# romi2002/gym-usv

Hardware: AMD Instinct MI355X
Metric: env-steps/sec at 65 536 parallel envs; 1/2/4/8 MI355X scaling (higher is better)
Workload: dtype f32; 1 GPU; C3: usv-simple, 65536 envs per GPU, random-action rollout, in-kernel TimeLimit + same-step autoreset; env_id=usv-simple, envs_per_gpu=65536, global_envs=65536, parallelism=env-sharded x1, no step-path collective, lidar=window

## Files before the change

gym-usv_amd/csrc/usv_kernels.hip:

```cpp
#include <hip/hip_runtime.h>

#include <algorithm>
#include <cstdio>
#include <type_traits>
#include <cstdlib>
#include <cstring>
#include <string>
#include <vector>

#include "usv_device.hpp"
#include "usv_hip.h"

namespace usv {

template <typename R> struct V4;
template <> struct V4<float> { typedef float T __attribute__((ext_vector_type(4))); };
template <> struct V4<double> { typedef double T __attribute__((ext_vector_type(4))); };
template <typename R> using R4 = typename V4<R>::T;

enum RealField {
  F_X, F_Y, F_PSI, F_U, F_V, F_R, F_LAST_U, F_LAST_R, F_PROGRESS,
  F_PX0, F_PY0, F_PX1, F_PY1, F_MAX_U, F_MAX_R, F_REF_V, F_NREAL
};

// ... 48 lines not shown
  }
}
constexpr int kExpN = 0, kExpPS = 1, kExpAngle = 3, kExpPose = 4, kExpObs = 8;

template <typename R> struct IO {
  const float* act;
  float* obs;
  R* rew;
  uint8_t* term;
  uint8_t* trunc;
  float* fobs;
  const uint8_t* mask;
  R* info;
  int kpath;
  uint8_t* done;
};

constexpr int kBlock = 256;
constexpr int kWaves = kBlock / kWave;
constexpr int kEPBReset = 64;
constexpr int kLidDefault = 7;

template <typename R> __device__ __forceinline__ R big() { return R(1e30); }

#ifdef USV_DIAG
#include "usv_diag.hpp"
#else
#define USV_STAMP_ID() do {} while (0)
#define USV_STAMP(i) do {} while (0)
#define USV_STAMP_B(i) do {} while (0)
#define USV_STAMP_W(i) do {} while (0)
#define USV_STAMP_V(i, v) do {} while (0)
struct Prof {
  __device__ void mark(int) {}
  __device__ void count(int) {}
  __device__ void flush(int) {}
};
struct QProf { __device__ void mark(int) {} __device__ void count(int, unsigned = 1) {} __device__ void flush() {} };
#define QMARK(i) do {} while (0)
#define QCOUNT(i, k) do {} while (0)
__device__ __forceinline__ void qprof_flush(QProf*) {}
#endif
template <typename T> __device__ __forceinline__ void st_out(T* p, T v) {
  __hip_atomic_store(p, v, __ATOMIC_RELAXED, __HIP_MEMORY_SCOPE_AGENT);
}
template <typename T> __device__ __forceinline__ void st_obs(T* p, T v) { st_out(p, v); }

constexpr int kRowSpanFrom = 196608;
constexpr int kStaticPrio = 1;

template <typename R> __device__ __forceinline__ R dyn_div(R a, R b) { return a / b; }
template <typename R> __device__ __forceinline__ R dyn_sqrt(R x) { return m_sqrt(x); }
template <> __device__ __forceinline__ float dyn_div(float a, float b) { return a * __builtin_amdgcn_rcpf(b); }
template <> __device__ __forceinline__ float dyn_sqrt(float x) { return __builtin_amdgcn_sqrtf(x); }

template <typename R> struct Vec2;
template <> struct Vec2<float> { using T = float2; };
template <> struct Vec2<double> { using T = double2; };

template <typename R> __device__ __forceinline__ R cdiv(R x, double c) { return div_const(x, c); }
template <> __device__ __forceinline__ float cdiv(float x, double c) { return x * (float)(1.0 / c); }

template <typename R>
__device__ __forceinline__ void make_header(float (&h)[kHdr], R u, R v, R r, R angle, R dist,
                                            R ye, R refv, R act_u, R act_r, R mu, R mr) {
  h[0] = (float)cdiv(u, 10); h[1] = (float)cdiv(v, 10); h[2] = (float)cdiv(r, 10);
  h[3] = (float)cdiv(angle, kPi); h[4] = (float)cdiv(dist, kDiag);
  h[5] = (float)cdiv(ye, 10); h[6] = (float)cdiv(refv, 10);
  h[7] = (float)dyn_div(act_u, mu); h[8] = (float)dyn_div(act_r, mr);
  h[9] = (float)cdiv(mu, 10); h[10] = 0.0f; h[11] = (float)cdiv(mr, 10);
  h[12] = (float)(kMaxAccU / 10.0); h[13] = 0.0f; h[14] = (float)(kMaxAccR / 10.0);
}

template <typename R> struct Uni4 { R u[4]; };
__device__ __forceinline__ void philox_uniforms(Philox& g, int l, Uni4<float>& o) {
  uint32_t a[4];
  g.c3 = (uint32_t)l;
  g.block(a[0], a[1], a[2], a[3]);
#pragma unroll
  for (int i = 0; i < 4; ++i) o.u[i] = (float)(a[i] >> 8) * (1.0f / 16777216.0f);
}
__device__ __forceinline__ void philox_uniforms(Philox& g, int l, Uni4<double>& o) {
  uint32_t a[4], b[4];
  g.c3 = (uint32_t)l;
  g.block(a[0], a[1], a[2], a[3]);
  g.c3 = (uint32_t)l + 64u;
  g.block(b[0], b[1], b[2], b[3]);
  const double k = 1.0 / 9007199254740992.0;
  o.u[0] = (double)((((uint64_t)a[0] << 32) | a[1]) >> 11) * k;
  o.u[1] = (double)((((uint64_t)a[2] << 32) | a[3]) >> 11) * k;
  o.u[2] = (double)((((uint64_t)b[0] << 32) | b[1]) >> 11) * k;
  o.u[3] = (double)((((uint64_t)b[2] << 32) | b[3]) >> 11) * k;
}

template <typename R>
__device__ __forceinline__ void reset_info(R* info, R x, R y, R psi, R u, R v, R r, R px0, R py0,
                                           R px1, R py1, R ye, R angle_n) {
  const R vals[USV_INFO_DIM] = {x, y, psi, u, v, r, px0, py0, px1, py1, R(0), R(0),
                                ye, angle_n, R(0), R(0), R(0), R(0), R(0), R(0), R(0), R(0)};
#pragma unroll
  for (int i = 0; i < USV_INFO_DIM; ++i) info[i] = vals[i];
}

template <typename R>
__device__ __forceinline__ R path_ye(R x, R y, R x0, R y0, R x1, R y1) {
  const R dx = x1 - x0, dy = y1 - y0;
  const R inv_len = R(1) / m_sqrt(dx * dx + dy * dy);
  return -(x - x0) * (dy * inv_len) + (y - y0) * (dx * inv_len);
}

template <typename R>
__device__ __forceinline__ void reset_experiment(const State<R>& S, int e, int ep, float* row, R* info) {
  const R* X = S.exp;
  R tx, ty, u, v, r, mu, mr, refv;
  {
    Philox g(S.seed, S.gid0 + (uint64_t)e, (uint32_t)ep);
    Uni4<R> U33, U34, U35;
    philox_uniforms(g, 33, U33);
    philox_uniforms(g, 34, U34);
    philox_uniforms(g, 35, U35);
    tx = R(kBound) * U33.u[1]; ty = R(kBound) * U33.u[2];
    u = R(0.15) * U33.u[3]; v = R(0.15) * U34.u[0]; r = R(0.15) * U34.u[1];
    mu = R(1.5) + R(1.5) * U34.u[2];
    mr = R(3) + R(3) * U34.u[3];
    refv = R(0.75) + (mu - R(0.75)) * U35.u[0];
  }
  const int cnt = (int)X[kExpN];
  R* ob = S.orow(e);
  for (int j = 0; j < S.cap; ++j) {
    ob[j] = j < cnt ? X[kExpObs + j] : R(0);
    ob[S.ostride + j] = j < cnt ? X[kExpObs + S.cap + j] : R(0);
    ob[2 * S.ostride + j] = j < cnt ? X[kExpObs + 2 * S.cap + j] : R(0);
  }
  const R ps0 = X[kExpPS], ps1 = X[kExpPS + 1];
  R sx2, cx2;
  m_sincos(X[kExpAngle], &sx2, &cx2);
  const R pe0 = ps0 + cx2 * R(100), pe1 = ps1 + sx2 * R(100);
  const R px = X[kExpPose], py = X[kExpPose + 1], psi = X[kExpPose + 2];
  S.F(F_X)[e] = px; S.F(F_Y)[e] = py;
  store_heading<R>(S, e, psi);
  S.F(F_PX0)[e] = ps0; S.F(F_PY0)[e] = ps1;
  S.F(F_PX1)[e] = pe0; S.F(F_PY1)[e] = pe1;
  S.I(I_NOBS)[e] = cnt;
  const R angle = wrap_angle(m_atan2(ty - py, tx - px) - psi);
  const R dst = m_hypot(px - tx, py - ty);
  const R ye = path_ye(px, py, ps0, ps1, pe0, pe1);
  float h[kHdr];
  make_header<R>(h, u, v, r, angle, dst, ye, refv, R(0), R(0), mu, mr);
  for (int i = 0; i < kHdr; ++i) row[i] = h[i];
  if (info) reset_info<R>(info, px, py, psi, u, v, r, ps0, ps1, pe0, pe1, ye, cdiv(angle, kPi));
}

template <typename R, int MODE>
__device__ __forceinline__ void reset_wave(const State<R>& S, int e, float* row, R* info = nullptr,
                                           int kpath = 0) {
  if (S.np_reset) return;
  const int l = lane_id();
  const int ep = uniform(S.I(I_EPISODE)[e]);
  Philox g(S.seed, S.gid0 + (uint64_t)e, (uint32_t)ep);
  Uni4<R> U;
  philox_uniforms(g, l, U);
  const R bm = m_sqrt(R(-2) * log(R(1) - bcast(U.u[0], 32)));
  R sb, cb;
  m_sincos(R(2 * kPi) * bcast(U.u[1], 32), &sb, &cb);
  const R sx = R(kBound / 2) + R(0.5) * bm * cb, sy = R(kBound / 2) + R(0.5) * bm * sb;
  const R tx = R(kBound) * bcast(U.u[1], 33), ty = R(kBound) * bcast(U.u[2], 33);
  const R mu = R(1.5) + R(1.5) * bcast(U.u[2], 34);
  const int n = min(15 + (int)(bcast(U.u[1], 35) * R(15)), 29);
  const R ox = R(kBound) * U.u[0], oy = R(kBound) * U.u[1], orad = R(0.15) + R(0.35) * U.u[2];
  const bool keep = (l < n) && !(m_hypot(sx - ox, sy - oy) < R(0.5) || m_hypot(tx - ox, ty - oy) < R(0.5));
  const unsigned long long ball = ballot(keep);
  int cnt = __popcll(ball);
  const int pos = __builtin_amdgcn_mbcnt_hi((unsigned)(ball >> 32), __builtin_amdgcn_mbcnt_lo((unsigned)ball, 0));
  R* ob = S.orow(e);
  const int os = S.ostride;
  if (keep) { ob[pos] = ox; ob[os + pos] = oy; ob[2 * os + pos] = orad; }
  if (cnt == 0) {
    const R fx = R(kBound) * bcast(U.u[2], 35), fy = R(kBound) * bcast(U.u[3], 35);
    const R fr = R(0.15) + R(0.35) * bcast(U.u[0], 36);
    if (l == 0) { ob[0] = fx; ob[os] = fy; ob[2 * os] = fr; }
    cnt = 1;
  }
  const R ang = R(-kPi) + R(2 * kPi) * bcast(U.u[3], 32);
  if (kpath > 0) {
    R sa, ca;
    m_sincos(ang, &sa, &ca);
    Uni4<R> P;
    philox_uniforms(g, l + 128, P);
    const R mag = R(kBound) * P.u[0];
    const R bq = m_sqrt(R(-2) * log(R(1) - P.u[1]));
    R s2, c2;
    m_sincos(R(2 * kPi) * P.u[2], &s2, &c2);
    const R lx = (ca * mag + sx) + bq * c2, ly = (sa * mag + sy) + bq * s2;
    const R lr = R(0.15) + R(0.35) * P.u[3];
    if (l < kpath) { ob[cnt + l] = lx; ob[os + cnt + l] = ly; ob[2 * os + cnt + l] = lr; }
    cnt += kpath;
  }
  if (l >= cnt && l < S.cap) { ob[l] = R(0); ob[os + l] = R(0); ob[2 * os + l] = R(0); }
  if (MODE == USV_MODE_ASMC_SIMPLE && l < kAsmcN) S.asmc[(size_t)l * S.N + e] = R(0);
  if (l == 0) {
    const R psi = R(-kPi) + R(2 * kPi) * bcast(U.u[2], 32);
    const R dist = R(100) + R(10) * bcast(U.u[0], 33);
    const R u = R(0.15) * bcast(U.u[3], 33), v = R(0.15) * bcast(U.u[0], 34), r = R(0.15) * bcast(U.u[1], 34);
    const R mr = R(3) + R(3) * bcast(U.u[3], 34);
    const R refv = R(0.75) + (mu - R(0.75)) * bcast(U.u[0], 35);
    R sa, ca;
    m_sincos(ang, &sa, &ca);
    S.F(F_X)[e] = sx; S.F(F_Y)[e] = sy;
    store_heading<R>(S, e, psi);
    S.F(F_U)[e] = u; S.F(F_V)[e] = v; S.F(F_R)[e] = r;
    S.F(F_PROGRESS)[e] = R(0);
    S.F(F_PX0)[e] = sx; S.F(F_PY0)[e] = sy;
    S.F(F_PX1)[e] = sx + ca * dist; S.F(F_PY1)[e] = sy + sa * dist;
    S.F(F_MAX_U)[e] = mu; S.F(F_MAX_R)[e] = mr; S.F(F_REF_V)[e] = refv;
    S.I(I_NOBS)[e] = cnt;
    S.I(I_ELAPSED)[e] = 0;
    S.I(I_EPISODE)[e] = ep + 1;
    S.I(I_SCAN)[e] = 0;
    const R angle = wrap_angle(m_atan2(ty - sy, tx - sx) - psi);
    const R dst = m_hypot(sx - tx, sy - ty);
    float h[kHdr];
    make_header<R>(h, u, v, r, angle, dst, R(0), refv, R(0), R(0), mu, mr);
#pragma unroll
    for (int i = 0; i < kHdr; ++i) row[i] = h[i];
    if (info) reset_info<R>(info, sx, sy, psi, u, v, r, sx, sy, sx + ca * dist, sy + sa * dist, R(0), cdiv(angle, kPi));
  }
}

template <typename R> __device__ __forceinline__ void heading_sincos(R psi, R* s, R* c) { fx_sincos(psi, s, c); }


#include "np_ziggurat.inc"
struct NpPcg64 {
  uint64_t sh, sl, ih, il;
  uint32_t has32, u32;
  __device__ uint64_t next64() {
    constexpr uint64_t kMh = 2549297995355413924ULL, kMl = 4865540595714422341ULL;
    const uint64_t lo = sl * kMl;
    const uint64_t hi = __umul64hi(sl, kMl) + sl * kMh + sh * kMl;
    const uint64_t nlo = lo + il;
    sh = hi + ih + (nlo < lo ? 1ULL : 0ULL);
    sl = nlo;
    const uint64_t x = sh ^ sl;
    const unsigned rot = (unsigned)(sh >> 58);
    return (x >> rot) | (x << ((64u - rot) & 63u));
  }
  __device__ uint32_t next32() {
    if (has32) { has32 = 0; return u32; }
    const uint64_t v = next64();
    has32 = 1;
    u32 = (uint32_t)(v >> 32);
    return (uint32_t)v;
  }
  __device__ double next_double() { return (double)(next64() >> 11) * (1.0 / 9007199254740992.0); }
  __device__ double standard_normal() {
    constexpr double kR = 3.6541528853610088, kInvR = 0.27366123732975828;
    for (;;) {
      uint64_t r = next64();
      const int idx = (int)(r & 0xff);
      r >>= 8;
      const bool neg = r & 1;
      const uint64_t rabs = (r >> 1) & 0x000fffffffffffffULL;
      double x = (double)rabs * kNpZigWi[idx];
      if (neg) x = -x;
      if (rabs < kNpZigKi[idx]) return x;
      if (idx == 0) {
        for (;;) {
          const double xx = -kInvR * log1p(-next_double());
          const double yy = -log1p(-next_double());
          if (yy + yy > xx * xx) return ((rabs >> 8) & 1) ? -(kR + xx) : kR + xx;
        }
      }
      if ((kNpZigFi[idx - 1] - kNpZigFi[idx]) * next_double() + kNpZigFi[idx] < exp(-0.5 * x * x)) return x;
    }
  }
  __device__ double uniform(double lo, double hi) { return lo + (hi - lo) * next_double(); }
  __device__ int integers(int lo, int hi) {
    const uint32_t rng = (uint32_t)(hi - 1 - lo), excl = rng + 1;
    uint64_t m = (uint64_t)next32() * excl;
    uint32_t left = (uint32_t)m;
    if (left < excl) {
      const uint32_t thr = (0xFFFFFFFFu - rng) % excl;
      while (left < thr) { m = (uint64_t)next32() * excl; left = (uint32_t)m; }
    }
    return lo + (int)(m >> 32);
  }
};

template <typename R>
__device__ __forceinline__ NpPcg64 np_load(const State<R>& S, int e) {
  auto w = [&](int i) { return (uint64_t)S.nprng[(size_t)i * S.fstride + e]; };
  return NpPcg64{w(0) | (w(1) << 32), w(2) | (w(3) << 32), w(4) | (w(5) << 32), w(6) | (w(7) << 32),
                 (uint32_t)w(8), (uint32_t)w(9)};
}
template <typename R>
__device__ __forceinline__ void np_store(const State<R>& S, int e, const NpPcg64& g) {
  const uint32_t v[10] = {(uint32_t)g.sh, (uint32_t)(g.sh >> 32), (uint32_t)g.sl, (uint32_t)(g.sl >> 32),
                          (uint32_t)g.ih, (uint32_t)(g.ih >> 32), (uint32_t)g.il, (uint32_t)(g.il >> 32),
                          g.has32, g.u32};
  for (int i = 0; i < 10; ++i) S.nprng[(size_t)i * S.fstride + e] = v[i];
}

template <typename R, int MODE>
__device__ void np_reset(const State<R>& S, int e, float* row, R* info = nullptr, int kpath = 0) {
  NpPcg64 g = np_load(S, e);
  const double sx = 0.5 * g.standard_normal() + kBound / 2;
  const double sy = 0.5 * g.standard_normal() + kBound / 2;
  (void)g.standard_normal(); (void)g.standard_normal(); (void)g.next_double();
  const double psi = g.uniform(-kPi, kPi);
  const double ang = g.uniform(-kPi, kPi), dist = g.uniform(100, 110);
  const double tx = g.uniform(0, kBound), ty = g.uniform(0, kBound);
  const double u = g.uniform(0.0, 0.15), v = g.uniform(0.0, 0.15), r = g.uniform(0.0, 0.15);
  const double mu = g.uniform(1.50, 3);
  (void)g.next_double(); (void)g.next_double();
  const double mr = g.uniform(3, 6);
  const double refv = g.uniform(0.75, mu);
  const int n = g.integers(15, 30);
  R* ob = S.orow(e);
  const int os = S.ostride;
  int cnt = 0;
  for (int j = 0; j < n; ++j) {
    const double ox = g.uniform(0, kBound), oy = g.uniform(0, kBound);
    if (!(hypot(sx - ox, sy - oy) < 0.5 || hypot(tx - ox, ty - oy) < 0.5)) {
      ob[cnt] = R(ox); ob[os + cnt] = R(oy); ++cnt;
    }
  }
  if (cnt == 0) {
    const double ox = g.uniform(0, kBound), oy = g.uniform(0, kBound);
    ob[0] = R(ox); ob[os] = R(oy); cnt = 1;
  }
  if (kpath > 0) {
    const double ca = cos(ang), sa = sin(ang);
    NpPcg64 gx = g, gy = g;
    for (int j = 0; j < kpath; ++j) (void)g.next_double();
    for (int j = 0; j < kpath; ++j) ob[cnt + j] = R((ca * gx.uniform(0, kBound) + sx) + g.standard_normal());
    for (int j = 0; j < kpath; ++j) ob[os + cnt + j] = R((sa * gy.uniform(0, kBound) + sy) + g.standard_normal());
    cnt += kpath;
  }
  for (int j = 0; j < cnt; ++j) ob[2 * os + j] = R(g.uniform(0.15, 0.5));
  np_store(S, e, g);
  double ps0 = sx, ps1 = sy, pe0 = sx + cos(ang) * dist, pe1 = sy + sin(ang) * dist;
  double px = sx, py = sy, pp = psi;
  if (const R* X = S.exp) {
    cnt = (int)X[kExpN];
    for (int j = 0; j < cnt; ++j) {
      ob[j] = X[kExpObs + j]; ob[os + j] = X[kExpObs + S.cap + j]; ob[2 * os + j] = X[kExpObs + 2 * S.cap + j];
    }
    ps0 = (double)X[kExpPS]; ps1 = (double)X[kExpPS + 1];
    pe0 = ps0 + cos((double)X[kExpAngle]) * 100; pe1 = ps1 + sin((double)X[kExpAngle]) * 100;
    px = (double)X[kExpPose]; py = (double)X[kExpPose + 1]; pp = (double)X[kExpPose + 2];
  }
  for (int j = cnt; j < S.cap; ++j) { ob[j] = R(0); ob[os + j] = R(0); ob[2 * os + j] = R(0); }
  if (MODE == USV_MODE_ASMC_SIMPLE)
    for (int i = 0; i < kAsmcN; ++i) S.asmc[(size_t)i * S.N + e] = R(0);
  const R x0 = R(px), y0 = R(py), ps = R(pp);
  S.F(F_X)[e] = x0; S.F(F_Y)[e] = y0;
  store_heading<R>(S, e, ps);
  S.F(F_U)[e] = R(u); S.F(F_V)[e] = R(v); S.F(F_R)[e] = R(r);
  S.F(F_PROGRESS)[e] = R(0);
  S.F(F_PX0)[e] = R(ps0); S.F(F_PY0)[e] = R(ps1);
  S.F(F_PX1)[e] = R(pe0); S.F(F_PY1)[e] = R(pe1);
  S.F(F_MAX_U)[e] = R(mu); S.F(F_MAX_R)[e] = R(mr); S.F(F_REF_V)[e] = R(refv);
  S.I(I_NOBS)[e] = cnt;
  S.I(I_ELAPSED)[e] = 0;
  S.I(I_EPISODE)[e] = S.I(I_EPISODE)[e] + 1;
  S.I(I_SCAN)[e] = 0;
  const R angle = wrap_angle(m_atan2(R(ty) - y0, R(tx) - x0) - ps);
  const R dst = m_hypot(x0 - R(tx), y0 - R(ty));
  const R ye = S.exp ? path_ye(x0, y0, R(ps0), R(ps1), R(pe0), R(pe1)) : R(0);
  float h[kHdr];
  make_header<R>(h, R(u), R(v), R(r), angle, dst, ye, R(refv), R(0), R(0), R(mu), R(mr));
  for (int i = 0; i < kHdr; ++i) row[i] = h[i];
  if (info) reset_info<R>(info, x0, y0, ps, R(u), R(v), R(r), R(ps0), R(ps1), R(pe0), R(pe1), ye, cdiv(angle, kPi));
}

template <typename R, int MODE>
__global__ __launch_bounds__(kBlock) void np_autoreset_kernel(State<R> S, IO<R> io) {
  const int e = blockIdx.x * kBlock + threadIdx.x;
  if (e >= S.N || !(io.term[e] | io.trunc[e])) return;
// ... 1009 lines not shown
  prof.mark(0);
  unsigned term_m, coll_m;
  scan_envs<R, MODE, LID>(S, io, L, e0, ne, P, nl, trunc_m, term_m, coll_m, prof);
  USV_STAMP_W(3);
  scan_epilogue<R, MODE>(S, io, e0, ne, R(0), false, term_m, coll_m, trunc_m);
  prof.mark(5);
  prof.flush(blockIdx.x * WPB + wave);
  USV_STAMP_W(6);
}

template <typename R, int MODE, int EPW, int LID, int WPB>
__global__ __launch_bounds__(kWave * WPB) __attribute__((amdgpu_num_sgpr(80), amdgpu_num_vgpr(64)))
void scan_kernel_tight(State<R> S, IO<R> io) { scan_body<R, MODE, EPW, LID, WPB>(S, io); }

template <typename R, int MODE, int EPW, int LID, int WPB>
__global__ __launch_bounds__(kWave * WPB) void scan_kernel(State<R> S, IO<R> io) {
  scan_body<R, MODE, EPW, LID, WPB>(S, io);
}

constexpr int kF64ScanWaves = 4;
template <typename R, int MODE, int EPW, int LID, int WPB>
__global__ __launch_bounds__(kWave * WPB) __attribute__((amdgpu_waves_per_eu(kF64ScanWaves, kF64ScanWaves)))
void scan_kernel_d(State<R> S, IO<R> io) { scan_body<R, MODE, EPW, LID, WPB>(S, io); }

template <typename R> __host__ __device__ constexpr size_t lds_blockdyn_bytes(int cap) {
  return (lds_scan_bytes<R>(cap) + 31) / 32 * 32 + 2 * kWave * sizeof(R4<R>);
}
template <typename R, int MODE, int EPW, int LID>
__device__ __forceinline__ void step_body_blockdyn(const State<R>& S, const IO<R>& io) {
  static_assert(kWaves * EPW <= kWave, "one dynamics lane per env of the block");
  extern __shared__ __attribute__((aligned(16))) char lds[];
  const int wave = __builtin_amdgcn_readfirstlane(threadIdx.x / kWave);
  const int l = lane_id();
  const int eb = blockIdx.x * kWaves * EPW;
  const int nbe = min(kWaves * EPW, S.N - eb);
  const int e0 = eb + wave * EPW;
  const int ne = min(EPW, S.N - e0);
  const ScanLds<R> L = scan_lds<R>(lds, wave, S.cap);
  R4<R>* const rec = reinterpret_cast<R4<R>*>(lds + (lds_scan_bytes<R>(S.cap) + 31) / 32 * 32);
  Prof prof;
  USV_STAMP_W(0);
  USV_STAMP_ID();
  if (S.prio == 1) __builtin_amdgcn_s_setprio(3);
  scan_prologue<R, LID>(S, L, wave, e0, ne);
  if (wave == 0) {
    const int e = eb + min(l, nbe - 1);
    const float2 a = reinterpret_cast<const float2*>(io.act)[e];
    const int nob = S.I(I_NOBS)[e];
    float hdr[kHdr];
    R px, py, sp, cp, partial;
    bool trunc;
    env_dynamics<R, MODE>(S, e, a.x, a.y, hdr, px, py, sp, cp, partial, trunc,
                          io.info ? io.info + (size_t)e * USV_INFO_DIM : nullptr);
    float* row = io.obs + (size_t)e * kObsDim;
#pragma unroll
    for (int i = 0; i < kHdr; ++i) row[i] = hdr[i];
    rec[l] = R4<R>{px, py, sp, cp};
    rec[kWave + l] = R4<R>{partial, R(nob), R(trunc ? 1 : 0), R(0)};
    USV_STAMP_W(1);
    if (io.fobs || S.autoreset == USV_AUTORESET_SAME_STEP) {
      __builtin_amdgcn_fence(__ATOMIC_RELEASE, "workgroup");
      vm_wait<0>();
    } else {
      vm_wait<2>();
    }
  } else {
    vm_wait<0>();
  }
  asm volatile("s_waitcnt lgkmcnt(0)\n\ts_barrier" ::: "memory");
  if (ne <= 0) return;
  USV_STAMP_W(2);
  prof.mark(0);
  const int k = wave * EPW + min(l, ne - 1);
  const R4<R> P = rec[k], M = rec[kWave + k];
  const unsigned trunc_m = (unsigned)ballot(M.z != R(0));
  unsigned term_m, coll_m;
  scan_envs<R, MODE, LID>(S, io, L, e0, ne, P, (int)M.y, trunc_m, term_m, coll_m, prof);
  USV_STAMP_W(3);
  scan_epilogue<R, MODE>(S, io, e0, ne, M.x, true, term_m, coll_m, trunc_m);
  prof.mark(5);
  prof.flush(blockIdx.x * kWaves + wave);
  USV_STAMP_W(6);
}

template <typename R, int MODE, int EPW, int LID>
__global__ __launch_bounds__(kBlock) __attribute__((amdgpu_waves_per_eu(kF64ScanWaves, kF64ScanWaves)))
void step_kernel_blockdyn(State<R> S, IO<R> io) { step_body_blockdyn<R, MODE, EPW, LID>(S, io); }

constexpr int kQSgpr = 80, kQWPE = 8;
constexpr int kQPrioDyn = 3, kQYoungWaves = 10;
constexpr int kQW = 16, kQE = 128, kQRec = 16;
__host__ __device__ constexpr size_t q_slice_bytes() { return 256 * 8 + 64 * 4 + 2 * 1024; }

__device__ __forceinline__ void dma_copy1(const void* src, void* dst, int bytes) {
  const int c = lane_id();
  const unsigned d = __builtin_amdgcn_readfirstlane((unsigned)(uintptr_t)dst);
  const uint64_t a = (uint64_t)(uintptr_t)src;
  const uint64_t sb = ((uint64_t)(unsigned)__builtin_amdgcn_readfirstlane((unsigned)(a >> 32)) << 32) |
                      (uint64_t)(unsigned)__builtin_amdgcn_readfirstlane((unsigned)a);
  if (c < bytes / 16) {
    unsigned keep;
    asm volatile("s_mov_b32 %0, m0\n\ts_mov_b32 m0, %3\n\ts_nop 0\n\t"
                 "global_load_lds_dwordx4 %1, %2\n\ts_mov_b32 m0, %0"
                 : "=&s"(keep) : "v"(16 * c), "s"(sb), "s"(d) : "memory");
  }
}

__device__ __forceinline__ void dma_copy_at(const void* base, int off, void* dst, int bytes) {
  const int c = lane_id();
  const unsigned d = __builtin_amdgcn_readfirstlane((unsigned)(uintptr_t)dst);
  const uint64_t a = (uint64_t)(uintptr_t)base;
  const uint64_t sb = ((uint64_t)(unsigned)__builtin_amdgcn_readfirstlane((unsigned)(a >> 32)) << 32) |
                      (uint64_t)(unsigned)__builtin_amdgcn_readfirstlane((unsigned)a);
  if (c < bytes / 16) {
    unsigned keep;
    asm volatile("s_mov_b32 %0, m0\n\ts_mov_b32 m0, %3\n\ts_nop 0\n\t"
                 "global_load_lds_dwordx4 %1, %2\n\ts_mov_b32 m0, %0"
                 : "=&s"(keep) : "v"(16 * c + off), "s"(sb), "s"(d) : "memory");
  }
}

__device__ __forceinline__ void make_qrec(float* rec, float px, float py, float sp, float cp, float partial,
                                          int n, bool trunc, const float (&h)[kHdr]) {
  const float c0 = ray_c(cp, sp, (float)kStartC, (float)kStartS), s0 = ray_s(cp, sp, (float)kStartC, (float)kStartS);
  float4* r4 = reinterpret_cast<float4*>(rec);
  r4[0] = make_float4(px, py, c0, s0);
  r4[1] = make_float4(partial, __int_as_float(n | (trunc ? 1 << 16 : 0)), h[0], h[2]);
  r4[2] = make_float4(h[3], h[4], h[5], h[6]);
  r4[3] = make_float4(h[7], h[8], h[9], h[11]);
}
__device__ __forceinline__ float qrec_hdr(const float* rec, int i) {
  const float v = rec[i == 0 ? 6 : (i <= 9 ? i + 5 : 15)];
  return (i == 1 || i == 10 || i == 13) ? 0.0f
       : i == 12 ? (float)(kMaxAccU / 10.0) : i == 14 ? (float)(kMaxAccR / 10.0) : v;
}

__device__ __forceinline__ void q_emit_done(const State<float>& S, const IO<float>& io, int e,
                                            const Scan<float>& sc, const float* rec, int rot) {
  const int l = lane_id();
  const int ray = (l - rot) & (kWave - 1);
  if (io.fobs) {
    float* f = io.fobs + (size_t)e * kObsDim;
    f[kHdr + ray] = l_norm(sc.rd0);
    f[kHdr + 64 + ray] = l_norm(sc.rd1);
    const int hi = min(l, kHdr - 1);
    f[hi] = qrec_hdr(rec, hi);
  }
  if (S.autoreset == USV_AUTORESET_SAME_STEP) {
    S.sensor_last[(size_t)e * kSensors + ray] = sc.rd0;
    S.sensor_last[(size_t)e * kSensors + 64 + ray] = sc.rd1;
  }
}

constexpr int kQE_S = 16, kQW_S = 8;
constexpr int kQSmallBelow = 32768;
template <int QE = kQE, int QW = kQW> __host__ __device__ constexpr size_t lds_q_bytes() {
  return wave_tab_bytes<float>() + QW * q_slice_bytes() + QE * kQRec * 4 + 16 + QE * 4;
}
static_assert(2 * lds_q_bytes() <= 160 * 1024, "two blocks per CU");
static_assert(4 * lds_q_bytes<kQE_S, kQW_S>() <= 160 * 1024, "four small blocks per CU");

template <int MODE, bool FUSED, bool DONE = false, int kQE = ::usv::kQE, int kQW = ::usv::kQW, bool CHAIN = true,
          bool INFO = false, bool SPAN = false>
__device__ __forceinline__ void step_q_body(const State<float>& S, const IO<float>& io) {
  extern __shared__ __attribute__((aligned(16))) char lds[];
  const int wave = __builtin_amdgcn_readfirstlane(threadIdx.x / kWave);
  const int l = lane_id();
  constexpr int os = 32, rowb = row_bytes<float>(32);
  const int eb = blockIdx.x * kQE;
  const int nbe = min(kQE, S.N - eb);
  const int np = (nbe + 1) >> 1;
  char* const slice = lds + wave_tab_bytes<float>() + wave * q_slice_bytes();
  unsigned long long* const slot = reinterpret_cast<unsigned long long*>(slice);
  int* const mark = reinterpret_cast<int*>(slice + 256 * 8);
  float* const rowbuf0 = reinterpret_cast<float*>(slice + 256 * 8 + 64 * 4);
  float* const rowbuf1 = rowbuf0 + 256;
  float* const recs = reinterpret_cast<float*>(lds + wave_tab_bytes<float>() + kQW * q_slice_bytes());
  unsigned* const qctr = reinterpret_cast<unsigned*>(recs + kQE * kQRec);
  int* const qnob = reinterpret_cast<int*>(recs + kQE * kQRec) + 4;
  const float2* const rayoff = reinterpret_cast<const float2*>(lds);
#ifdef USV_DIAG_QPROF
  QProf qprof;
  QProf* const qp = &qprof;
#else
  QProf* const qp = nullptr;
#endif
  unsigned* const qdyn = qctr + 1;
  if (threadIdx.x == 0) {
    qctr[0] = kQW;
    qdyn[0] = 0u;
    qdyn[1] = 0u;
  }

  if (wave == kQW - 1) dma_copy(S.ray_tab, lds, (int)wave_tab_bytes<float>());
#pragma unroll
  for (int i = 0; i < 4; ++i) slot[i * 64 + l] = kSlotArm;
  mark[l] = 0;
  USV_STAMP_W(0);
  USV_STAMP_ID();
  int cur = wave < np ? wave : -1;
  constexpr int kDynWaves = FUSED ? (kQE + kWave - 1) / kWave : 0;
  static_assert(kQW >= 3 * kDynWaves + 1 && 2 * kQW <= kQE + 2 * kWave, "block shape");
  static_assert(kDynWaves <= 2, "qdyn holds two dynamics waves' flags");
  if (wave >= kDynWaves && cur >= 0) dma_copy1(S.orow(eb + 2 * cur), rowbuf0, min(2, nbe - 2 * cur) * rowb);
  if (FUSED && wave >= kDynWaves && wave < 2 * kDynWaves) {
    const int w = wave - kDynWaves;
    if (w < np)
      dma_copy1(S.orow(eb + 2 * w), lds + wave_tab_bytes<float>() + w * q_slice_bytes() + 256 * 8 + 64 * 4,
                min(2, nbe - 2 * w) * rowb);
  }
  if constexpr (FUSED) {
    if (wave >= 2 * kDynWaves && wave < 3 * kDynWaves) {
      const int k = (wave - 2 * kDynWaves) * kWave + l;
      if (k < nbe) qnob[k] = S.I(I_NOBS)[eb + k];
    }
    if (wave < kDynWaves && wave * kWave < nbe) {
      if (S.qyoung != INT_MAX) __builtin_amdgcn_s_setprio(kQPrioDyn);
      const int k = min(wave * kWave + l, nbe - 1);
      const int e = eb + k;
      const float2 a = reinterpret_cast<const float2*>(io.act)[e];
      float hdr[kHdr];
      float px, py, sp, cp, partial;
      bool trunc;
      env_dynamics<float, MODE, CHAIN>(S, e, a.x, a.y, hdr, px, py, sp, cp, partial, trunc,
                                       INFO ? io.info + (size_t)e * USV_INFO_DIM : nullptr);
      io.trunc[e] = trunc;
      make_qrec(recs + k * kQRec, px, py, sp, cp, partial, 0, trunc, hdr);
    }
  } else {
    if (wave < kQE / 16 && wave * 16 < nbe)
      dma_copy1(S.qrec + (size_t)(eb + wave * 16) * kQRec, recs + wave * 16 * kQRec, min(16, nbe - wave * 16) * kQRec * 4);
  }
  USV_STAMP_W(1);
  if (wave >= kDynWaves) vm_wait<0>();
  QMARK(10);
  asm volatile("s_waitcnt lgkmcnt(0)\n\ts_barrier" ::: "memory");
  if (FUSED && wave < kDynWaves) __builtin_amdgcn_s_setprio(0);
  if ((int)blockIdx.x >= S.qyoung && wave < kQYoungWaves) __builtin_amdgcn_s_setprio(1);
  if (FUSED && wave < kDynWaves) {
    vm_wait<0>();
    __hip_atomic_store(qdyn + wave, 1u, __ATOMIC_RELEASE, __HIP_MEMORY_SCOPE_WORKGROUP);
  }
  USV_STAMP_W(2);
  QMARK(0);
  unsigned tk = 0;
  if (l == 0) tk = atomicAdd(qctr, 1u);
  int it = 0;
#ifdef USV_DIAG_STAMPS
  unsigned wsum = 0;
#endif
  const bool hb = l >= 32;
  auto pair_hasb = [&](int p) { return 2 * p + 1 < nbe; };
  const float* const oblk = S.orow(eb);

  const unsigned ob = (unsigned)(((uintptr_t)io.obs >> 2) & 7);
  auto pair_shift = [&](int p) { return (int)((ob + (unsigned)(eb + 2 * p) * (unsigned)kObsDim) & 7u); };
  int hpk = 0;
  if constexpr (!SPAN) {
    const int hl = min(l, 2 * kHdr - 1);
    const int hi = hl >= kHdr ? hl - kHdr : hl;
    const int hrec = hi == 0 ? 6 : (hi <= 9 ? hi + 5 : 15);
    hpk = hi | (hrec << 8) | ((hl >= kHdr) << 16) | ((hi == 1 || hi == 10 || hi >= 12) << 17);
  }
  auto rec_of = [&](int c, float4& P, float4& M, float& H) {
    const int c0 = 2 * c;
    const bool cB = pair_hasb(c);
    const int kk = (hb && cB) ? c0 + 1 : c0;
    const float* const rk = recs + kk * kQRec;
    P = *reinterpret_cast<const float4*>(rk);
    M = *reinterpret_cast<const float4*>(rk + 4);
    if constexpr (FUSED) M.y = __int_as_float(__float_as_int(M.y) | qnob[kk]);
    if constexpr (!SPAN) {
      H = recs[((((hpk >> 16) & 1) && cB) ? c0 + 1 : c0) * kQRec + ((hpk >> 8) & 31)];
      return;
    }
    const int hl = min(max(l - ((SPAN && cB) ? pair_shift(c) : 0), 0), 2 * kHdr - 1);
    const int hi = hl >= kHdr ? hl - kHdr : hl;
    float v = recs[((hl >= kHdr && cB) ? c0 + 1 : c0) * kQRec + (hi == 0 ? 6 : (hi <= 9 ? hi + 5 : 15))];
    const bool cst = ((0x7402 >> hi) & 1) != 0;
    const float hc = hi == 12 ? (float)(kMaxAccU / 10.0) : (hi == 14 ? (float)(kMaxAccR / 10.0) : 0.0f);
    asm volatile("" : "+v"(v));
    H = cst ? hc : v;
  };
  for (;;) {
    unsigned done = 0;
    int de0 = 0;
    float4 pose = make_float4(0.f, 0.f, 0.f, 0.f), meta = pose;
    float hv = 0.0f;
    if (cur >= 0) rec_of(cur, pose, meta, hv);
    while (cur >= 0) {
      int nxt = (int)__builtin_amdgcn_readlane(tk, 0);
      QCOUNT(8, 1);
      const bool odd = (it & 1) != 0;
      float* const cbuf = odd ? rowbuf1 : rowbuf0;
      float* const nbuf = odd ? rowbuf0 : rowbuf1;
      const int k0 = 2 * cur;
      const int e0 = eb + k0;
      const bool hasB = pair_hasb(cur);
      if (nxt >= np) nxt = -1;
      if (nxt >= 0) {
        if (l == 0) tk = atomicAdd(qctr, 1u);
        dma_copy_at(oblk, 2 * rowb * nxt, nbuf, (pair_hasb(nxt) ? 2 : 1) * rowb);
      }
      const int kl = (hb && hasB) ? k0 + 1 : k0;
      const int el = e0 + (kl - k0);
      const int nt = __float_as_int(meta.y);
      const bool span2 = SPAN && hasB;
      const int sh = span2 ? pair_shift(cur) : 0;
      const int rotA = span2 ? kHdr + sh : 0, rotB = span2 ? 2 * kHdr + sh : 0;
      Scan<float> sa, sb;
      QMARK(1);
#ifdef USV_DIAG_STAMPS
      int wq = 0;
      lidar_wave2(cbuf, os, (hb && !hasB) ? 0 : (nt & 0xffff), pose.x, pose.y, pose.z, pose.w, rayoff, slot,
                  mark, reinterpret_cast<int*>(nbuf) + 192, sa, sb, qp, rotA, rotB, &wq);
      wsum += (unsigned)wq;
#else
      lidar_wave2(cbuf, os, (hb && !hasB) ? 0 : (nt & 0xffff), pose.x, pose.y, pose.z, pose.w, rayoff, slot,
                  mark, reinterpret_cast<int*>(nbuf) + 192, sa, sb, qp, rotA, rotB);
#endif
      float4 pose_n = pose, meta_n = meta;
      float hv_n = hv;
      if (nxt >= 0) rec_of(nxt, pose_n, meta_n, hv_n);
      const float kc = (float)kCollDist;
      const bool collA = (ballot(sa.rd0 < kc) | ballot(sa.rd1 < kc)) != 0;
      const bool collB = hasB ? (ballot(sb.rd0 < kc) | ballot(sb.rd1 < kc)) != 0 : collA;
      const bool termB = hasB ? sb.term : sa.term;
      float* const rowA = io.obs + (size_t)e0 * kObsDim;
      if (span2) {
        float* const span = rowA - sh;
        const float a0 = l_norm(sa.rd0), a1 = l_norm(sa.rd1), b0 = l_norm(sb.rd0), b1 = l_norm(sb.rd1);
        const bool mA = l < kHdr + sh, mB = l < 2 * kHdr + sh;
        if (l >= sh) st_obs(span + l, mA ? hv : a0);
        st_obs(span + 64 + l, mA ? a0 : a1);
        st_obs(span + 128 + l, mA ? a1 : (mB ? hv : b0));
        st_obs(span + 192 + l, mB ? b0 : b1);
        if (mB) st_obs(span + 256 + l, b1);
      } else {
        {
        float* const rowB = rowA + (hasB ? kObsDim : 0);
        st_obs(rowA + kHdr + l, l_norm(sa.rd0));
        st_obs(rowA + kHdr + 64 + l, l_norm(sa.rd1));
        st_obs(rowB + kHdr + l, l_norm(hasB ? sb.rd0 : sa.rd0));
        st_obs(rowB + kHdr + 64 + l, l_norm(hasB ? sb.rd1 : sa.rd1));
        if constexpr (SPAN) {
          const int hl = min(l, 2 * kHdr - 1);
          st_obs((hl >= kHdr ? rowB - kHdr : rowA) + hl, hv);
        } else {
          const int hi = hpk & 31;
          const bool hB = ((hpk >> 16) & 1) && hasB;
          const float hc = hi == 12 ? (float)(kMaxAccU / 10.0) : hi == 14 ? (float)(kMaxAccR / 10.0) : 0.0f;
          st_obs(rowA + (hB ? kObsDim : 0) + hi, ((hpk >> 17) & 1) ? hc : hv);
        }
        }
      }
      const bool term_l = hb ? termB : sa.term;
      const bool coll_l = hb ? collB : collA;
      st_out(io.rew + el, coll_l ? -20.0f + meta.x : meta.x);
      io.term[el] = term_l;
      const bool done_l = term_l | ((nt >> 16) & 1);
      if constexpr (DONE) io.done[el] = done_l;
      const unsigned long long dm = ballot(done_l);
      const bool doneA = (unsigned)dm != 0u, doneB = hasB && (unsigned)(dm >> 32) != 0u;
      if (doneA | doneB) {
        if (doneA) q_emit_done(S, io, e0, sa, recs + k0 * kQRec, rotA);
        if (doneB) q_emit_done(S, io, e0 + 1, sb, recs + (k0 + 1) * kQRec, rotB);
      }
      QMARK(5);
      vm_wait<7>();
      QMARK(6);
      if (it == 0) USV_STAMP_W(5);
      cur = nxt;
      pose = pose_n;
      meta = meta_n;
      hv = hv_n;
      ++it;
      if (S.autoreset == USV_AUTORESET_SAME_STEP && (doneA | doneB)) {
        done = (doneA ? 1u : 0u) | (doneB ? 2u : 0u);
        de0 = e0;
        break;
      }
    }
    if (!done) break;
    QMARK(11);
    for (; done; done &= done - 1) {
      const int e = de0 + __builtin_ctz(done);
      if constexpr (FUSED) {
        const unsigned* const f = qdyn + ((e - eb) >> 6);
        while (__hip_atomic_load(f, __ATOMIC_ACQUIRE, __HIP_MEMORY_SCOPE_WORKGROUP) == 0u)
          __builtin_amdgcn_s_sleep(2);
      }
      reset_wave<float, MODE>(S, e, io.obs + (size_t)e * kObsDim);
    }
    QMARK(7);
  }
  QMARK(11);
  qprof_flush(qp);
#ifdef USV_DIAG_STAMPS
  USV_STAMP_V(4, (unsigned long long)it | ((unsigned long long)wsum << 16));
#endif
  USV_STAMP_W(3);
  USV_STAMP_W(6);
}

template <int MODE, bool FUSED, bool DONE, bool CHAIN = true, bool INFO = false, bool SPAN = false>
__global__ __launch_bounds__(kQW * kWave) __attribute__((amdgpu_num_sgpr(kQSgpr), amdgpu_waves_per_eu(kQWPE, kQWPE)))
void step_q_kernel(State<float> S, IO<float> io) { step_q_body<MODE, FUSED, DONE, kQE, kQW, CHAIN, INFO, SPAN>(S, io); }
template <int MODE, bool DONE, bool CHAIN = true, bool INFO = false>
__global__ __launch_bounds__(kQW_S * kWave) __attribute__((amdgpu_num_sgpr(80), amdgpu_waves_per_eu(8, 8)))
void step_qs_kernel(State<float> S, IO<float> io) { step_q_body<MODE, true, DONE, kQE_S, kQW_S, CHAIN, INFO>(S, io); }

template <int MODE>
__global__ __launch_bounds__(kBlock) __attribute__((amdgpu_waves_per_eu(1, 2))) void dyn_rec_kernel(State<float> S, IO<float> io) {
  const int e = blockIdx.x * kBlock + threadIdx.x;
  if (e >= S.N) return;
  const float2 a = reinterpret_cast<const float2*>(io.act)[e];
  const int nob = S.I(I_NOBS)[e];
  float hdr[kHdr];
  float px, py, sp, cp, partial;
  bool trunc;
  env_dynamics<float, MODE>(S, e, a.x, a.y, hdr, px, py, sp, cp, partial, trunc,
                            io.info ? io.info + (size_t)e * USV_INFO_DIM : nullptr);
  io.trunc[e] = trunc;
  make_qrec(S.qrec + (size_t)e * kQRec, px, py, sp, cp, partial, nob, trunc, hdr);
}

template <typename R>
__global__ __launch_bounds__(kBlock) __attribute__((amdgpu_waves_per_eu(1, 2))) void asmc_chain_kernel(State<R> S, IO<R> io) {
  const int e = blockIdx.x * kBlock + threadIdx.x;
  if (e >= S.N) return;
  const float2 a = reinterpret_cast<const float2*>(io.act)[e];
  R x = S.F(F_X)[e], y = S.F(F_Y)[e], psi = S.F(F_PSI)[e];
  R u = S.F(F_U)[e], v = S.F(F_V)[e], r = S.F(F_R)[e];
  asmc_env_chain<R>(S, e, S.I(I_ELAPSED)[e], a.x, a.y, x, y, psi, u, v, r);
  S.F(F_X)[e] = x; S.F(F_Y)[e] = y; S.F(F_PSI)[e] = psi;
  S.F(F_U)[e] = u; S.F(F_V)[e] = v; S.F(F_R)[e] = r;
}

template <typename R, int MODE>
__global__ __launch_bounds__(kBlock) void reset_kernel(State<R> S, IO<R> io) {
  extern __shared__ __attribute__((aligned(16))) char lds[];
  auto* rayoff = reinterpret_cast<typename Vec2<R>::T*>(lds);
  auto* slots = reinterpret_cast<unsigned long long*>(lds + lds_rayoff_bytes<R>());
  const int tid = threadIdx.x;
  const int wave = __builtin_amdgcn_readfirstlane(tid / kWave);
  const int l = lane_id();
  const int e0 = blockIdx.x * kEPBReset;
  const int ne = S.N - e0 < kEPBReset ? S.N - e0 : kEPBReset;
  int* marks = reinterpret_cast<int*>(lds + lds_rayoff_bytes<R>() + kLdsSlotBytes);
  R* wx = reinterpret_cast<R*>(lds + lds_head_bytes<R>()) + wave * 3 * 64;
  R* wy = wx + 64;
  R* wr = wy + 64;
  lds_prologue(S, lds, tid);
  __syncthreads();
  for (int k = wave; k < ne; k += kWaves) {
    const int e = e0 + k;
    if (io.mask && !io.mask[e]) continue;
    R rd0, rd1;
    R* last = S.sensor_last + (size_t)e * kSensors;
    if (S.I(I_SCAN)[e]) {
      R sp, cp;
      heading_sincos(S.F(F_PSI)[e], &sp, &cp);
      const int n = uniform(S.I(I_NOBS)[e]);
      if (l < S.cap) {
        const R* o = S.orow(e);
        wx[l] = o[l]; wy[l] = o[S.ostride + l]; wr[l] = o[2 * S.ostride + l];
      }
      Scan<R> sc;
      lidar_wave<R, kLidDefault>(RowSoA<R>{wx, wy, wr}, n, S.F(F_X)[e], S.F(F_Y)[e], sp, cp, rayoff,
                                 slots + wave * 128, marks + wave * 64, sc);
      rd0 = sc.rd0;
      rd1 = sc.rd1;
      last[l] = rd0;
      last[64 + l] = rd1;
    } else {
      rd0 = last[l];
      rd1 = last[64 + l];
    }
    float* row = io.obs + (size_t)e * kObsDim;
    row[kHdr + l] = (float)l_norm(rd0);
    row[kHdr + 64 + l] = (float)l_norm(rd1);
    R* info = io.info ? io.info + (size_t)e * USV_INFO_DIM : nullptr;
    if (S.np_reset) {
      if (l == 0) np_reset<R, MODE>(S, e, row, info, io.kpath);
    } else {
      const int ep = uniform(S.I(I_EPISODE)[e]);
      reset_wave<R, MODE>(S, e, row, info, io.kpath);
      if (S.exp) {
        __threadfence_block();
        if (l == 0) reset_experiment<R>(S, e, ep, row, info);
      }
    }
  }
}

constexpr double kV0MinSpeed = 0.3, kV0KAk = 5.72, kV0KYe = 0.5, kV0SigmaYe = 1.0;
constexpr double kV0CAction = 1.0 / (((kPi / 2) / 2 - (-kPi / 2) / 2) / H * (((kPi / 2) / 2 - (-kPi / 2) / 2) / H));
constexpr double kV0WAction = 0.2, kV0TMin = -30.0, kV0TMax = 36.5;
constexpr int kFamV0 = 0, kFamYeInt = 1, kFamPid = 2;

template <typename R> __device__ __forceinline__ R q32(R x) { return R((float)x); }

template <typename R> __device__ __forceinline__ void v0_path_sincos(R ak, R& sa, R& ca) {
  if (__builtin_amdgcn_ballot_w64(ak != R(0)) == 0) { sa = R(0); ca = R(1); }
  else { sa = m_sin(ak); ca = m_cos(ak); }
}

template <typename R>
__device__ __forceinline__ void v0_obs(float* row, R u, R v_ak, R r, R ye, R psi_ak, R a_last) {
  row[0] = (float)u; row[1] = (float)v_ak; row[2] = (float)r;
  row[3] = (float)ye; row[4] = (float)psi_ak; row[5] = (float)a_last;
}

struct NpMt {
  uint32_t* k;
  size_t stride;
  __device__ uint32_t& key(int i) const { return k[(size_t)i * stride]; }
  __device__ void twist() const {
    constexpr uint32_t kA = 0x9908b0dfu, kU = 0x80000000u, kL = 0x7fffffffu;
    int i = 0;
    for (; i < 624 - 397; ++i) {
      const uint32_t y = (key(i) & kU) | (key(i + 1) & kL);
      key(i) = key(i + 397) ^ (y >> 1) ^ ((0u - (y & 1u)) & kA);
    }
    for (; i < 623; ++i) {
      const uint32_t y = (key(i) & kU) | (key(i + 1) & kL);
      key(i) = key(i + 397 - 624) ^ (y >> 1) ^ ((0u - (y & 1u)) & kA);
    }
    const uint32_t y = (key(623) & kU) | (key(0) & kL);
    key(623) = key(396) ^ (y >> 1) ^ ((0u - (y & 1u)) & kA);
    key(624) = 0;
  }
  __device__ uint32_t next32() const {
    if (key(624) >= 624) twist();
    const uint32_t p = key(624);
    key(624) = p + 1;
    uint32_t y = key((int)p);
    y ^= y >> 11;
    y ^= (y << 7) & 0x9d2c5680u;
    y ^= (y << 15) & 0xefc60000u;
    y ^= y >> 18;
    return y;
  }
  __device__ double uniform(double lo, double hi) const {
    const uint32_t a = next32() >> 5, b = next32() >> 6;
// ... 1118 lines not shown
```

gym-usv_amd/gym_usv_amd/build.py:

```python
from __future__ import annotations

import os
import subprocess
import sys

PKG = os.path.dirname(os.path.abspath(__file__))
ROOT = os.path.dirname(os.path.dirname(PKG))
CSRC = os.path.join(os.path.dirname(PKG), "csrc")
INCLUDE = os.path.join(ROOT, "include")
ARCH = os.environ.get("USV_OFFLOAD_ARCH", "gfx950")


DEVICE_FLAGS = ["-mllvm", "-amdgpu-atomic-optimizer-strategy=None"]


def hipcc():
    for c in (os.environ.get("HIPCC"), "/opt/rocm/bin/hipcc", "hipcc"):
        if c and (os.path.isabs(c) and os.path.exists(c) or not os.path.isabs(c)):
            return c
    raise RuntimeError("hipcc not found")


def sources():
    return [os.path.join(CSRC, "usv_kernels.hip")]


def deps():
    return sources() + [os.path.join(CSRC, f) for f in os.listdir(CSRC) if f.endswith((".hpp", ".h", ".inc"))] + \
        [os.path.join(INCLUDE, "usv_hip.h")]


VARIANTS = {"product": ("libusvhip.so", []), "safe": ("libusvhip_safe.so", ["-DUSV_SAFE_VMCNT"])}


def _stale(out):
    return not os.path.exists(out) or any(os.path.getmtime(d) > os.path.getmtime(out) for d in deps())


def _cmd(variant):
    name, defs = VARIANTS[variant]
    out = os.path.join(PKG, name)
    return out, [hipcc(), "-O3", f"--offload-arch={ARCH}", "-std=c++17", "-fPIC", "-shared", "-Wall",
                 *DEVICE_FLAGS, *defs, f"-I{INCLUDE}", "-o", out + ".tmp"] + sources()


def build_library(force=False, verbose=True, variant="product"):
    out, cmd = _cmd(variant)
    if not force and not _stale(out):
        return out
    if verbose:
        print(" ".join(cmd), flush=True)
    subprocess.run(cmd, check=True)
    os.replace(out + ".tmp", out)
    return out


def build_all(force=False, verbose=True):
    jobs = []
    for v in VARIANTS:
        out, cmd = _cmd(v)
        if force or _stale(out):
            if verbose:
                print(" ".join(cmd), flush=True)
            jobs.append((out, subprocess.Popen(cmd)))
    failed = []
    for out, p in jobs:
        if p.wait() == 0:
            os.replace(out + ".tmp", out)
        else:
            failed.append((p.returncode, out))
            if os.path.exists(out + ".tmp"):
                os.remove(out + ".tmp")
    if failed:
        rc, out = failed[0]
        raise subprocess.CalledProcessError(rc, "hipcc " + out)


if __name__ == "__main__":
    build_all(force="--force" in sys.argv)
```

Baseline: 3.487 billion env-steps/s.

## Move cold done/reset path off hot loop registers via kernarg reload and LDS-staged episodes

Prefetches per-env episode counters into LDS during block setup and moves hot-loop setup (header packing, obstacle block pointer) into a lambda run after the DMA waits. The rare done/reset branches are marked cold with expect_with_probability and reload State/IO from the kernarg segment, so the hot loop does not keep those values live in SGPRs. Compiler flags stop LLVM from hoisting code into hotter blocks. The aim is lower register pressure and a tighter inner ray-cast loop, at the cost of a little extra LDS and dependence on compiler block-frequency heuristics.

```diff
diff --git a/gym-usv_amd/csrc/usv_kernels.hip b/gym-usv_amd/csrc/usv_kernels.hip
--- a/gym-usv_amd/csrc/usv_kernels.hip
+++ b/gym-usv_amd/csrc/usv_kernels.hip
@@ -224,11 +224,10 @@
 }
 
 template <typename R, int MODE>
-__device__ __forceinline__ void reset_wave(const State<R>& S, int e, float* row, R* info = nullptr,
-                                           int kpath = 0) {
+__device__ __forceinline__ void reset_wave_ep(const State<R>& S, int e, int ep, float* row, R* info = nullptr,
+                                              int kpath = 0) {
   if (S.np_reset) return;
   const int l = lane_id();
-  const int ep = uniform(S.I(I_EPISODE)[e]);
   Philox g(S.seed, S.gid0 + (uint64_t)e, (uint32_t)ep);
   Uni4<R> U;
   philox_uniforms(g, l, U);
@@ -297,6 +296,13 @@
     for (int i = 0; i < kHdr; ++i) row[i] = h[i];
     if (info) reset_info<R>(info, sx, sy, psi, u, v, r, sx, sy, sx + ca * dist, sy + sa * dist, R(0), cdiv(angle, kPi));
   }
+}
+
+template <typename R, int MODE>
+__device__ __forceinline__ void reset_wave(const State<R>& S, int e, float* row, R* info = nullptr,
+                                           int kpath = 0) {
+  if (S.np_reset) return;
+  reset_wave_ep<R, MODE>(S, e, uniform(S.I(I_EPISODE)[e]), row, info, kpath);
 }
 
 template <typename R> __device__ __forceinline__ void heading_sincos(R psi, R* s, R* c) { fx_sincos(psi, s, c); }
@@ -1612,10 +1618,22 @@
   }
 }
 
+constexpr double kQRare = 1.0 - 1e-6;
+struct QColdArgs { State<float> S; IO<float> io; };
+static_assert(sizeof(State<float>) % alignof(IO<float>) == 0, "IO follows State in the kernarg segment");
+__device__ __forceinline__ QColdArgs q_cold_args() {
+  typedef const __attribute__((address_space(4))) QColdArgs* KArg;
+  KArg ka = (KArg)__builtin_amdgcn_kernarg_segment_ptr();
+  asm volatile("" : "+s"(ka));
+  QColdArgs c;
+  __builtin_memcpy(&c, ka, sizeof(c));
+  return c;
+}
+
 constexpr int kQE_S = 16, kQW_S = 8;
 constexpr int kQSmallBelow = 32768;
 template <int QE = kQE, int QW = kQW> __host__ __device__ constexpr size_t lds_q_bytes() {
-  return wave_tab_bytes<float>() + QW * q_slice_bytes() + QE * kQRec * 4 + 16 + QE * 4;
+  return wave_tab_bytes<float>() + QW * q_slice_bytes() + QE * kQRec * 4 + 16 + 2 * QE * 4;
 }
 static_assert(2 * lds_q_bytes() <= 160 * 1024, "two blocks per CU");
 static_assert(4 * lds_q_bytes<kQE_S, kQW_S>() <= 160 * 1024, "four small blocks per CU");
@@ -1638,6 +1656,7 @@
   float* const recs = reinterpret_cast<float*>(lds + wave_tab_bytes<float>() + kQW * q_slice_bytes());
   unsigned* const qctr = reinterpret_cast<unsigned*>(recs + kQE * kQRec);
   int* const qnob = reinterpret_cast<int*>(recs + kQE * kQRec) + 4;
+  int* const qep = qnob + kQE;
   const float2* const rayoff = reinterpret_cast<const float2*>(lds);
 #ifdef USV_DIAG_QPROF
   QProf qprof;
@@ -1669,11 +1688,19 @@
       dma_copy1(S.orow(eb + 2 * w), lds + wave_tab_bytes<float>() + w * q_slice_bytes() + 256 * 8 + 64 * 4,
                 min(2, nbe - 2 * w) * rowb);
   }
+  {
+    constexpr int kStageWaves = (kQE + kWave - 1) / kWave;
+    constexpr int kStage0 = FUSED ? 2 * kDynWaves : kQW - 1 - kStageWaves;
+    static_assert(kStage0 >= kDynWaves && kStage0 + kStageWaves <= kQW, "staging waves");
+    if (wave >= kStage0 && wave < kStage0 + kStageWaves) {
+      const int k = (wave - kStage0) * kWave + l;
+      if (k < nbe) {
+        if constexpr (FUSED) qnob[k] = S.I(I_NOBS)[eb + k];
+        qep[k] = S.I(I_EPISODE)[eb + k];
+      }
+    }
+  }
   if constexpr (FUSED) {
-    if (wave >= 2 * kDynWaves && wave < 3 * kDynWaves) {
-      const int k = (wave - 2 * kDynWaves) * kWave + l;
-      if (k < nbe) qnob[k] = S.I(I_NOBS)[eb + k];
-    }
     if (wave < kDynWaves && wave * kWave < nbe) {
       if (S.qyoung != INT_MAX) __builtin_amdgcn_s_setprio(kQPrioDyn);
       const int k = min(wave * kWave + l, nbe - 1);
@@ -1691,6 +1718,22 @@
     if (wave < kQE / 16 && wave * 16 < nbe)
       dma_copy1(S.qrec + (size_t)(eb + wave * 16) * kQRec, recs + wave * 16 * kQRec, min(16, nbe - wave * 16) * kQRec * 4);
   }
+  int hpk = 0;
+  const float* oblk = nullptr;
+  unsigned ob = 0;
+  auto loop_setup = [&] {
+    if constexpr (!SPAN) {
+      const int hl = min(l, 2 * kHdr - 1);
+      const int hi = hl >= kHdr ? hl - kHdr : hl;
+      const int hrec = hi == 0 ? 6 : (hi <= 9 ? hi + 5 : 15);
+      hpk = hi | (hrec << 8) | ((hl >= kHdr) << 16) | ((hi == 1 || hi == 10 || hi >= 12) << 17);
+      asm volatile("" : "+v"(hpk));
+    }
+    oblk = S.orow(eb);
+    ob = (unsigned)(((uintptr_t)io.obs >> 2) & 7);
+    asm volatile("" : "+s"(oblk), "+s"(ob));
+  };
+  if (wave >= kDynWaves) loop_setup();
   USV_STAMP_W(1);
   if (wave >= kDynWaves) vm_wait<0>();
   QMARK(10);
@@ -1700,6 +1743,7 @@
   if (FUSED && wave < kDynWaves) {
     vm_wait<0>();
     __hip_atomic_store(qdyn + wave, 1u, __ATOMIC_RELEASE, __HIP_MEMORY_SCOPE_WORKGROUP);
+    loop_setup();
   }
   USV_STAMP_W(2);
   QMARK(0);
@@ -1711,17 +1755,8 @@
 #endif
   const bool hb = l >= 32;
   auto pair_hasb = [&](int p) { return 2 * p + 1 < nbe; };
-  const float* const oblk = S.orow(eb);
-
-  const unsigned ob = (unsigned)(((uintptr_t)io.obs >> 2) & 7);
+
   auto pair_shift = [&](int p) { return (int)((ob + (unsigned)(eb + 2 * p) * (unsigned)kObsDim) & 7u); };
-  int hpk = 0;
-  if constexpr (!SPAN) {
-    const int hl = min(l, 2 * kHdr - 1);
-    const int hi = hl >= kHdr ? hl - kHdr : hl;
-    const int hrec = hi == 0 ? 6 : (hi <= 9 ? hi + 5 : 15);
-    hpk = hi | (hrec << 8) | ((hl >= kHdr) << 16) | ((hi == 1 || hi == 10 || hi >= 12) << 17);
-  }
   auto rec_of = [&](int c, float4& P, float4& M, float& H) {
     const int c0 = 2 * c;
     const bool cB = pair_hasb(c);
@@ -1822,9 +1857,10 @@
       if constexpr (DONE) io.done[el] = done_l;
       const unsigned long long dm = ballot(done_l);
       const bool doneA = (unsigned)dm != 0u, doneB = hasB && (unsigned)(dm >> 32) != 0u;
-      if (doneA | doneB) {
-        if (doneA) q_emit_done(S, io, e0, sa, recs + k0 * kQRec, rotA);
-        if (doneB) q_emit_done(S, io, e0 + 1, sb, recs + (k0 + 1) * kQRec, rotB);
+      if (__builtin_expect_with_probability(doneA | doneB, 0, kQRare)) {
+        const QColdArgs c = q_cold_args();
+        if (doneA) q_emit_done(c.S, c.io, e0, sa, recs + k0 * kQRec, rotA);
+        if (doneB) q_emit_done(c.S, c.io, e0 + 1, sb, recs + (k0 + 1) * kQRec, rotB);
       }
       QMARK(5);
       vm_wait<7>();
@@ -1835,14 +1871,15 @@
       meta = meta_n;
       hv = hv_n;
       ++it;
-      if (S.autoreset == USV_AUTORESET_SAME_STEP && (doneA | doneB)) {
+      if (__builtin_expect_with_probability(S.autoreset == USV_AUTORESET_SAME_STEP && (doneA | doneB), 0, kQRare)) {
         done = (doneA ? 1u : 0u) | (doneB ? 2u : 0u);
         de0 = e0;
         break;
       }
     }
-    if (!done) break;
+    if (__builtin_expect(!done, 1)) break;
     QMARK(11);
+    const QColdArgs c = q_cold_args();
     for (; done; done &= done - 1) {
       const int e = de0 + __builtin_ctz(done);
       if constexpr (FUSED) {
@@ -1850,7 +1887,7 @@
         while (__hip_atomic_load(f, __ATOMIC_ACQUIRE, __HIP_MEMORY_SCOPE_WORKGROUP) == 0u)
           __builtin_amdgcn_s_sleep(2);
       }
-      reset_wave<float, MODE>(S, e, io.obs + (size_t)e * kObsDim);
+      reset_wave_ep<float, MODE>(c.S, e, uniform(qep[e - eb]), c.io.obs + (size_t)e * kObsDim);
     }
     QMARK(7);
   }
diff --git a/gym-usv_amd/gym_usv_amd/build.py b/gym-usv_amd/gym_usv_amd/build.py
--- a/gym-usv_amd/gym_usv_amd/build.py
+++ b/gym-usv_amd/gym_usv_amd/build.py
@@ -11,7 +11,8 @@
 ARCH = os.environ.get("USV_OFFLOAD_ARCH", "gfx950")
 
 
-DEVICE_FLAGS = ["-mllvm", "-amdgpu-atomic-optimizer-strategy=None"]
+DEVICE_FLAGS = ["-mllvm", "-amdgpu-atomic-optimizer-strategy=None",
+                "-mllvm", "-disable-hoisting-to-hotter-blocks=all", "-mllvm", "-block-freq-ratio-threshold=1"]
 
 
 def hipcc():
```

Result: faster. 3.576 billion env-steps/s, median of 6 (+2.6%).
